# kakaobrain/rq-vae-transformer

Measured on AMD Instinct MI355X. Metric: 256x256 images/sec, AR sampling + decode (RQ-Transformer huge, 8x8x4 codes), higher is better.
Workload: dtype bf16

## Files before the change

### rq-vae-transformer_amd/csrc/conv_halo.hip

```cpp
#include <stdlib.h>
#include <type_traits>
#include "gemm.h"
#include "rq_common.h"
#include "vae_kernels.h"
#ifndef RQ_CONV_NT
#define RQ_CONV_NT 0
#endif
#ifndef RQ_CONVOUT_NT
#define RQ_CONVOUT_NT 0
#endif
static __device__ __forceinline__ rq_u128 ld128_act(const void* p) {
#if RQ_CONV_NT >= 2
    return ld128_nt(p);
#else
    return ld128(p);
#endif
}
static __device__ __forceinline__ void st128_act(void* p, rq_u128 v) {
#if RQ_CONV_NT >= 1
    st128_nt(p, v);
#else
    st128(p, v);
#endif
}
// ... 816 lines not shown
                for (int k = 0; k < PPT; ++k) {
                    const int it = (tap - FIRST) * PPT + k;
                    if (ptap && it < H_IT) rh[it] = halo_piece_value(rh, it);
                }
                compute(hbuf, wbuf, ky, kx, rh, -1);
            }
            store_w(wbuf ^ 1, rw[(tap + 1) % W_SETS]);
#pragma unroll
            for (int k = 0; k < PPT; ++k) {
                const int it = (tap - FIRST) * PPT + k;
                if (!(ptap && it < H_IT)) continue;
                if (h_in(it)) st128(sH + (hbuf ^ 1) * PK_PSTRIDE + h_loff(it), rh[it]);
            }
            RQ_CTP(2 + (c * 9 + tap) * 2);
            rq_syncthreads();
            RQ_CTP(3 + (c * 9 + tap) * 2);
            wbuf ^= 1;
        }
        hbuf ^= 1;
    };

    for (;;) {
        rq_opaque(tid_o);
        static_assert(CPR == 16 && NTH / CPR == HT_W && R_IT == TH, "piece k = tile row k");
        if (SUB)
            io_off0 = (unsigned)((((long)cur.img * p.H + 2 * cur.ty0 + (cur.cls >> 1)) * p.W + 2 * (cur.tx0 + (tid_o >> 4)) + (cur.cls & 1)) * p.Cout + cur.n0 + (tid_o & 15) * 8) * 2u;
        else
            io_off0 = (unsigned)((((long)cur.img * p.H + cur.ty0) * p.W + cur.tx0 + (tid_o >> 4)) * p.Cout + cur.n0 + (tid_o & 15) * 8) * 2u;
        RQ_CTP(1);
        for (int c = 0; c + 1 < NC; ++c) run_chunk(c, std::false_type{});
        run_chunk(NC - 1, std::true_type{});

        char* sT = (char*)smem + PK_P0 + (hbuf == 0 ? PK_PATCH : 0);
        const int lane_o = tid_o & 63, wave_o = tid_o >> 6, wm_o = wave_o >> 1, wn_o = wave_o & 1;
        float* sred = (float*)(sT + PK_TILE);
        if (RES) {
#pragma unroll
            for (int k = 0; k < R_IT; ++k) st128(sT + ((tid_o >> 4) + HT_W * k) * PK_LDR + (tid_o & 15) * 16, rr[k]);
            rq_syncthreads();
        }
#pragma unroll
        for (int i = 0; i < RPW; ++i) {
            const int ty = wm_o * RPW + i, tx = lane_o & 31;
            const int ml = ty * HT_W + tx;
#pragma unroll
            for (int j = 0; j < 2; ++j) {
#pragma unroll
                for (int q = 0; q < 4; ++q) {
                    const int nl = wn_o * 64 + j * 32 + 8 * q + 4 * (lane_o >> 5);
                    float v[4];
#pragma unroll
                    for (int e = 0; e < 4; ++e) v[e] = acc[i][j][4 * q + e];
                    if (RES) {
                        const uint32_t* rp = (const uint32_t*)(sT + ml * PK_LDR + nl * 2);
                        const uint32_t r0 = rp[0], r1 = rp[1];
                        { float lo_, hi_; rq_unpack2(r0, lo_, hi_); v[0] += lo_; v[1] += hi_; }
                        { float lo_, hi_; rq_unpack2(r1, lo_, hi_); v[2] += lo_; v[3] += hi_; }
                    }
                    struct __attribute__((aligned(8))) u64 { uint32_t a, b; } w2;
                    w2.a = pack_bf16x2(v[0], v[1]);
                    w2.b = pack_bf16x2(v[2], v[3]);
                    *(u64*)(sT + ml * PK_LDR + nl * 2) = w2;
                }
            }
        }
        if (has_next) acc_from_bias(nxt.n0);
        rq_syncthreads();
        RQ_CTP(61);
        float gs_[4], gq_[4];
#pragma unroll
        for (int e = 0; e < 4; ++e) { gs_[e] = 0.f; gq_[e] = 0.f; }
#pragma unroll
        for (int k = 0; k < R_IT; ++k) {
            const rq_u128 u = ld128(sT + ((tid_o >> 4) + HT_W * k) * PK_LDR + (tid_o & 15) * 16);
            st128_act((char*)p.out + (io_off0 + (unsigned)k * io_step), u);
            if (p.stats) rq_stats_piece(u, gs_, gq_);
        }
        if (p.stats) {
            const int gsz = p.Cout / 32;
            float a0, q0, a1, q1;
            if (gsz == 4) {
                a0 = gs_[0] + gs_[1]; q0 = gq_[0] + gq_[1];
                a1 = gs_[2] + gs_[3]; q1 = gq_[2] + gq_[3];
            } else {
                a0 = (gs_[0] + gs_[1]) + (gs_[2] + gs_[3]);
                q0 = (gq_[0] + gq_[1]) + (gq_[2] + gq_[3]);
                a1 = 0.f; q1 = 0.f;
            }
            a0 += rq_shfl_xor(a0, 16); q0 += rq_shfl_xor(q0, 16); a1 += rq_shfl_xor(a1, 16); q1 += rq_shfl_xor(q1, 16);
            a0 += rq_shfl_xor(a0, 32); q0 += rq_shfl_xor(q0, 32); a1 += rq_shfl_xor(a1, 32); q1 += rq_shfl_xor(q1, 32);
            if (lane_o < 16) {
                float* o = sred + (wave_o * 16 + lane_o) * 4;
                o[0] = a0; o[1] = q0; o[2] = a1; o[3] = q1;
            }
            rq_syncthreads();
            if (wave_o == 0) {
                const int chunk = (lane_o >> 1) & 15, pair = lane_o & 1;
                float a = 0.f, q = 0.f;
#pragma unroll
                for (int w = 0; w < NTH / 64; ++w) { a += sred[(w * 16 + chunk) * 4 + pair * 2]; q += sred[(w * 16 + chunk) * 4 + pair * 2 + 1]; }
                if (gsz == 16) {
                    a += rq_shfl_xor(a, 2);
                    q += rq_shfl_xor(q, 2);
                }
                const bool writer = gsz == 4 ? true : (gsz == 8 ? pair == 0 : (pair == 0 && (chunk & 1) == 0));
                if (writer && lane_o < 32) {
                    const int g = (cur.n0 + chunk * 8 + pair * 4) / gsz;
                    const int tiles = tiles_x * tiles_y * NCLS;
                    float* o = p.stats + (((long)cur.img * tiles + cur.trem) * 32 + g) * 2;
                    o[0] = a;
                    o[1] = q;
                }
            }
        }
        RQ_CTP(63);
#ifdef RQ_CONV_TRACE
        ++trace_tile;
#endif
        if (!has_next) break;
        rq_use(rw[1][0].x, rw[1][1].x, rw[2][0].x, rw[2][1].x);
        if (SUB) rq_use(rw[W_SETS - 1][0].x, rw[W_SETS - 1][1].x, rw[W_SETS - 1][0].y, rw[W_SETS - 1][1].y);
        rq_use(acc[0][0][0], acc[RPW - 1][1][15]);
        slot += wpx;
        cur = nxt;
        wn_cur = wn_nxt;
        if (SUB) set_class(cur.cls);
        has_next = slot_ok(slot + wpx);
        if (has_next) { nxt = decode(slot + wpx); wn_nxt = (unsigned)nxt.n0 * w_per_n + (unsigned)nxt.cls * w_per_cls; }
    }
}

struct ConvOutArgs {
    const bf16_t* x;
    const float* w;
    const float* bias;
    const float* gn;
    float* y;
    int B, H, W, Cin, Cout;
};
constexpr int OT_H = 4, OP_N = (OT_H + 2) * HP_W;
constexpr int O_NTH = 256;
constexpr int O_PLANE = OP_N * 128;

template <int FUSE_GN>
__global__ __launch_bounds__(O_NTH) void conv_out_halo_kernel(ConvOutArgs p) {
    RQ_DYN_SMEM(smem);
    const int NC = p.Cin / 64;
    char* sH = (char*)smem;
    const int wrow = 9 * p.Cin * 2 + 32;
    char* sW = sH + NC * O_PLANE;
    const int tid = threadIdx.x, lane = tid & 63, wave = rq_uniform(tid >> 6);

    const int tiles_x = p.W / HT_W, tiles_y = p.H / OT_H, tiles_img = tiles_x * tiles_y;
    const int n_mt = p.B * tiles_img;
    const int id = blockIdx.x, xcd = id & 7, slot = id >> 3, S = (int)gridDim.x >> 3;
    const int per = (n_mt + 7) >> 3;
    const int x0 = xcd * per, x1 = x0 + per < n_mt ? x0 + per : n_mt;
    const int sub = (x1 - x0 + S - 1) / (S > 0 ? S : 1);
    const int t0 = x0 + slot * sub, t1 = t0 + sub < x1 ? t0 + sub : x1;
    if (x0 >= x1 || t0 >= t1) return;

    const int cpp_sh = p.Cin == 64 ? 3 : 4;
    const int CPP = 1 << cpp_sh;
    const int cq = tid & (CPP - 1);
    const int n_piece = OP_N << cpp_sh;
    constexpr int PIT = 13;
    unsigned hyx[PIT];
#pragma unroll
    for (int k = 0; k < PIT; ++k) {
        const int q = tid + O_NTH * k;
        const int hp = q >> cpp_sh;
        const int hy = hp / HP_W, hx = hp - hy * HP_W;
        hyx[k] = q < n_piece ? (unsigned)(hy << 8 | hx) : 0xffffu;
    }
    const char* gX = (const char*)p.x;
    struct Tile { int img, ty0, tx0; };
    auto decode = [&](int t) {
        Tile d;
        d.img = t / tiles_img;
        const int trem = t - d.img * tiles_img;
        d.ty0 = (trem / tiles_x) * OT_H;
        d.tx0 = (trem - (trem / tiles_x) * tiles_x) * HT_W;
        return d;
    };
    auto request = [&](const Tile& d, rq_u128* r, f32x4* gs) {
        if (FUSE_GN) {
            const float* gn = p.gn + ((long)d.img * p.Cin + cq * 8) * 2;
#pragma unroll
            for (int e = 0; e < 4; ++e) gs[e] = *(const f32x4*)(gn + e * 4) * RQ_LOG2E;
        }
#pragma unroll
        for (int k = 0; k < PIT; ++k) {
            if (hyx[k] == 0xffffu) continue;
            const int gy = d.ty0 + (int)(hyx[k] >> 8) - 1, gx = d.tx0 + (int)(hyx[k] & 255u) - 1;
            const int cy = gy < 0 ? 0 : (gy >= p.H ? p.H - 1 : gy), cx = gx < 0 ? 0 : (gx >= p.W ? p.W - 1 : gx);
#if RQ_CONVOUT_NT
            r[k] = ld128_nt(gX + ((((long)d.img * p.H + cy) * p.W + cx) * p.Cin + cq * 8) * 2);
#else
            r[k] = ld128(gX + ((((long)d.img * p.H + cy) * p.W + cx) * p.Cin + cq * 8) * 2);
#endif
        }
    };
    auto stage = [&](const Tile& d, const rq_u128* r, const f32x4* gs) {
#pragma unroll
        for (int k = 0; k < PIT; ++k) {
            if (hyx[k] == 0xffffu) continue;
            const int hy = (int)(hyx[k] >> 8), hx = (int)(hyx[k] & 255u);
            const int gy = d.ty0 + hy - 1, gx = d.tx0 + hx - 1;
            rq_u128 v = r[k];
            if (FUSE_GN) {
                float f[8];
                rq_unpack2(v.x, f[0], f[1]);
                rq_unpack2(v.y, f[2], f[3]);
                rq_unpack2(v.z, f[4], f[5]);
                rq_unpack2(v.w, f[6], f[7]);
#pragma unroll
                for (int e = 0; e < 8; e += 2) {
                    const f32x4 ss = gs[e >> 1];
                    const float a = fmaf(f[e], ss[0], ss[1]), b = fmaf(f[e + 1], ss[2], ss[3]);
                    f[e] = rq_silu_l2(a);
                    f[e + 1] = rq_silu_l2(b);
                }
                v.x = pack_bf16x2(f[0], f[1]); v.y = pack_bf16x2(f[2], f[3]);
                v.z = pack_bf16x2(f[4], f[5]); v.w = pack_bf16x2(f[6], f[7]);
            }
            if (gy < 0 || gy >= p.H || gx < 0 || gx >= p.W) v = zero128();
            st128(sH + (unsigned)((cq >> 3) * O_PLANE) + halo_lds_off(hy, hx, cq & 7), v);
        }
    };

    rq_u128 r[PIT];
    f32x4 gs[4];
    Tile cur = decode(t0);
    request(cur, r, gs);
    const int KT = 9 * p.Cin;
    const int n_w4 = p.Cout * (KT >> 2);
    constexpr int WIT = 5;
    {
        f32x4 wr[WIT];
#pragma unroll
        for (int k = 0; k < WIT; ++k) {
            const int i = tid + O_NTH * k;
            if (i < n_w4) wr[k] = *(const f32x4*)(p.w + (long)i * 4);
        }
        stage(cur, r, gs);
#pragma unroll
        for (int k = 0; k < WIT; ++k) {
            const int i = tid + O_NTH * k;
            if (i < n_w4) {
                const int row = i / (KT >> 2), k4 = (i - row * (KT >> 2)) * 4;
                *(uint64_t*)(sW + row * wrow + k4 * 2) = (uint64_t)pack_bf16x2(wr[k][0], wr[k][1]) | ((uint64_t)pack_bf16x2(wr[k][2], wr[k][3]) << 32);
            }
        }
        for (int i = n_w4 + tid; i < 8 * (KT >> 2); i += O_NTH) {
            const int row = i / (KT >> 2), k4 = (i - row * (KT >> 2)) * 4;
            *(uint64_t*)(sW + row * wrow + k4 * 2) = 0ull;
        }
    }

    const int ftx = lane & 31, fk = lane >> 5;
    const char* wl = sW + (ftx & 7) * wrow + fk * 16;
    float bias_r[4];
#pragma unroll
    for (int co = 0; co < 4; ++co) bias_r[co] = co < p.Cout ? p.bias[co] : 0.f;
    for (int t = t0; t < t1; ++t) {
        const bool more = t + 1 < t1;
        Tile nxt = cur;
        if (more) { nxt = decode(t + 1); request(nxt, r, gs); }
        rq_syncthreads();
        f32x16 acc;
#pragma unroll
        for (int q = 0; q < 16; ++q) acc[q] = 0.f;
        constexpr int OD = 4;
        for (int c = 0; c < NC; ++c) {
            bf16x8 af[OD + 1], wf[OD + 1];
            auto frag = [&](int s, bf16x8& a, bf16x8& w) {
                const int tap = s >> 2, ks = s & 3, ky = tap / 3, kx = tap - ky * 3;
                const unsigned ha = (unsigned)(c * O_PLANE) + halo_lds_off(wave + ky, ftx + kx, fk);
                a = as_bf16x8(ld128(sH + (ha ^ (unsigned)(ks << 5))));
                w = as_bf16x8(ld128(wl + (tap * p.Cin + c * 64) * 2 + ks * 32));
            };
#pragma unroll
            for (int s = 0; s < OD; ++s) frag(s, af[s], wf[s]);
#pragma unroll
            for (int s = 0; s < 36; ++s) {
                if (s + OD < 36) frag(s + OD, af[(s + OD) % (OD + 1)], wf[(s + OD) % (OD + 1)]);
                acc = rq_mfma_32x32x16_bf16(wf[s % (OD + 1)], af[s % (OD + 1)], acc);
                rq_sched_barrier();
            }
        }
        if (lane < 32) {
            const int oy = cur.ty0 + wave, ox = cur.tx0 + lane;
#pragma unroll
            for (int co = 0; co < 4; ++co)
                if (co < p.Cout) p.y[(((long)cur.img * p.Cout + co) * p.H + oy) * p.W + ox] = acc[co] + bias_r[co];
        }
        if (!more) break;
        rq_syncthreads();
        stage(nxt, r, gs);
        cur = nxt;
    }
}

bool rq_conv_out_halo_supported(int H, int W, int Cin, int Cout) {
    return H % OT_H == 0 && W % HT_W == 0 && (Cin == 64 || Cin == 128) && Cout >= 1 && Cout <= 4;
}

int rq_launch_conv_out_halo(const bf16_t* x, const float* w, const float* bias, const float* gn, float* y, int B, int H, int W,
                            int Cin, int Cout, hipStream_t s) {
    if (!rq_conv_out_halo_supported(H, W, Cin, Cout)) return rq_fail(RQAMD_ERR_UNSUPPORTED, "conv_out_halo: shape %dx%d %d->%d", H, W, Cin, Cout);
    ConvOutArgs a{};
    a.x = x; a.w = w; a.bias = bias; a.gn = gn; a.y = y; a.B = B; a.H = H; a.W = W; a.Cin = Cin; a.Cout = Cout;
    const size_t smem = (size_t)(Cin / 64) * O_PLANE + 8 * (size_t)(9 * Cin * 2 + 32);
    static RqDeviceOnce attr_once;
    if (attr_once.first()) {
        (void)hipFuncSetAttribute((const void*)conv_out_halo_kernel<0>, hipFuncAttributeMaxDynamicSharedMemorySize, 160 * 1024);
        (void)hipFuncSetAttribute((const void*)conv_out_halo_kernel<1>, hipFuncAttributeMaxDynamicSharedMemorySize, 160 * 1024);
    }
    const int n_mt = B * (H / OT_H) * (W / HT_W);
    int nblocks = 8 * ((n_mt + 7) / 8);
    int cus = 256;
    (void)hipDeviceGetAttribute(&cus, hipDeviceAttributeMultiprocessorCount, 0);
    if (nblocks > 2 * cus) nblocks = 2 * cus / 8 * 8;
    if (const char* e = getenv("RQAMD_CONV_OUT_WGS")) {
        const int v = atoi(e) / 8 * 8;
        if (v >= 8 && v < nblocks) nblocks = v;
    }
    if (gn) RQ_LAUNCH(conv_out_halo_kernel<1>, dim3(nblocks), dim3(O_NTH), smem, s, a);
    else RQ_LAUNCH(conv_out_halo_kernel<0>, dim3(nblocks), dim3(O_NTH), smem, s, a);
    return rq_check_launch("conv_out_halo_kernel");
}

struct ConvInArgs {
    const float* x;
    const float* w;
    const float* bias;
    bf16_t* y;
    float* stats;
    int B, H, W;
};
constexpr int CI_COUT = 128, CI_PATCH = 3 * (HT_H + 2) * HP_W;
constexpr int CI_WROW = 80;
constexpr int CI_STG = 32 * (CI_COUT * 2 + 16);

__global__ __launch_bounds__(256) void conv_in_mfma_kernel(ConvInArgs p) {
    RQ_DYN_SMEM(smem);
    float* sP = (float*)smem;
    int* sK = (int*)(smem + 4096);
    char* sWt = (char*)smem + 4096 + 128;
    char* sO = sWt + CI_COUT * CI_WROW;
    const int tid = threadIdx.x, lane = tid & 63, wave = rq_uniform(tid >> 6);
    const int tiles_x = p.W / HT_W, tiles_y = p.H / HT_H;
    const int tile = blockIdx.x;
    const int img = tile / (tiles_y * tiles_x), trem = tile - img * (tiles_y * tiles_x);
    const int ty0 = (trem / tiles_x) * HT_H, tx0 = (trem - (trem / tiles_x) * tiles_x) * HT_W;

    for (int i = tid; i < CI_PATCH + 4; i += 256) {
        float v = 0.f;
        if (i < CI_PATCH) {
            const int ci = i / ((HT_H + 2) * HP_W), r = i - ci * ((HT_H + 2) * HP_W);
            const int hy = r / HP_W, hx = r - hy * HP_W;
            const int gy = ty0 + hy - 1, gx = tx0 + hx - 1;
            if (gy >= 0 && gy < p.H && gx >= 0 && gx < p.W) v = p.x[(((long)img * 3 + ci) * p.H + gy) * p.W + gx];
        }
        sP[i] = v;
    }
    if (tid < 32) {
        const int k = tid, tap = k / 3, ci = k - tap * 3, ky = tap / 3, kx = tap - ky * 3;
        sK[k] = k < 27 ? ci * ((HT_H + 2) * HP_W) + ky * HP_W + kx : -1;
    }
    for (int i = tid; i < CI_COUT * 16; i += 256) {
        const int co = i >> 4, k2 = (i & 15) * 2;
        const float a = k2 < 27 ? p.w[k2 * CI_COUT + co] : 0.f, b = k2 + 1 < 27 ? p.w[(k2 + 1) * CI_COUT + co] : 0.f;
        *(uint32_t*)(sWt + co * CI_WROW + k2 * 2) = pack_bf16x2(a, b);
    }
    rq_syncthreads();

    const int px = lane & 31, g = lane >> 5;
    int koff[2][8];
#pragma unroll
    for (int ks = 0; ks < 2; ++ks)
#pragma unroll
        for (int e = 0; e < 8; ++e) koff[ks][e] = sK[ks * 16 + g * 8 + e];
    bf16x8 bfr[2][4];
#pragma unroll
    for (int ks = 0; ks < 2; ++ks)
#pragma unroll
        for (int j = 0; j < 4; ++j) bfr[ks][j] = as_bf16x8(ld128(sWt + (j * 32 + px) * CI_WROW + (ks * 16 + g * 8) * 2));
    char* stg = sO + wave * CI_STG;
    float gs_[4] = {0.f, 0.f, 0.f, 0.f}, gq_[4] = {0.f, 0.f, 0.f, 0.f};
#pragma unroll 1
    for (int i = 0; i < 2; ++i) {
        const int row = wave * 2 + i;
        f32x16 acc[4];
#pragma unroll
        for (int j = 0; j < 4; ++j)
#pragma unroll
            for (int r = 0; r < 16; ++r) acc[j][r] = 0.f;
#pragma unroll
        for (int ks = 0; ks < 2; ++ks) {
            float f[8];
#pragma unroll
            for (int e = 0; e < 8; ++e) f[e] = koff[ks][e] >= 0 ? sP[koff[ks][e] + row * HP_W + px] : 0.f;
            rq_u128 u;
            u.x = pack_bf16x2(f[0], f[1]); u.y = pack_bf16x2(f[2], f[3]);
            u.z = pack_bf16x2(f[4], f[5]); u.w = pack_bf16x2(f[6], f[7]);
            const bf16x8 af = as_bf16x8(u);
#pragma unroll
            for (int j = 0; j < 4; ++j) acc[j] = rq_mfma_32x32x16_bf16(bfr[ks][j], af, acc[j]);
        }
#pragma unroll
        for (int j = 0; j < 4; ++j)
#pragma unroll
            for (int q = 0; q < 4; ++q) {
                const int co = j * 32 + 8 * q + 4 * g;
                const f32x4 bv = *(const f32x4*)(p.bias + co);
                struct __attribute__((aligned(8))) u64 { uint32_t a, b; } w2;
                w2.a = pack_bf16x2(acc[j][4 * q] + bv[0], acc[j][4 * q + 1] + bv[1]);
                w2.b = pack_bf16x2(acc[j][4 * q + 2] + bv[2], acc[j][4 * q + 3] + bv[3]);
                *(u64*)(stg + px * (CI_COUT * 2 + 16) + co * 2) = w2;
            }
        rq_syncthreads();
        const long pix0 = ((long)img * p.H + ty0 + row) * p.W + tx0;
#pragma unroll
        for (int k = 0; k < 8; ++k) {
            const int c = lane + 64 * k, opx = c >> 4, part = c & 15;
            const rq_u128 u = ld128(stg + opx * (CI_COUT * 2 + 16) + part * 16);
            st128(p.y + (pix0 + opx) * CI_COUT + part * 8, u);
            if (p.stats) rq_stats_piece(u, gs_, gq_);
        }
        rq_syncthreads();
    }
    if (p.stats) {
        float a0 = gs_[0] + gs_[1], q0 = gq_[0] + gq_[1], a1 = gs_[2] + gs_[3], q1 = gq_[2] + gq_[3];
        a0 += rq_shfl_xor(a0, 16); q0 += rq_shfl_xor(q0, 16); a1 += rq_shfl_xor(a1, 16); q1 += rq_shfl_xor(q1, 16);
        a0 += rq_shfl_xor(a0, 32); q0 += rq_shfl_xor(q0, 32); a1 += rq_shfl_xor(a1, 32); q1 += rq_shfl_xor(q1, 32);
        float* sred = (float*)sO;
        if (lane < 16) {
            float* o = sred + (wave * 16 + lane) * 4;
            o[0] = a0; o[1] = q0; o[2] = a1; o[3] = q1;
        }
        rq_syncthreads();
        if (tid < 32) {
            const int chunk = tid >> 1, pair = tid & 1;
            float a = 0.f, q = 0.f;
#pragma unroll
            for (int w = 0; w < 4; ++w) { a += sred[(w * 16 + chunk) * 4 + pair * 2]; q += sred[(w * 16 + chunk) * 4 + pair * 2 + 1]; }
            float* o = p.stats + (((long)img * (tiles_y * tiles_x) + trem) * 32 + tid) * 2;
            o[0] = a;
            o[1] = q;
        }
    }
}

bool rq_conv_in_mfma_supported(int H, int W, int Cin, int Cout) {
    return Cin == 3 && Cout == CI_COUT && H % HT_H == 0 && W % HT_W == 0;
}

int rq_launch_conv_in_mfma(const float* x, const float* w, const float* bias, bf16_t* y, float* stats, int B, int H, int W, hipStream_t s) {
    ConvInArgs a{};
    a.x = x; a.w = w; a.bias = bias; a.y = y; a.stats = stats; a.B = B; a.H = H; a.W = W;
    const size_t smem = 4096 + 128 + (size_t)CI_COUT * CI_WROW + 4 * (size_t)CI_STG;
    static RqDeviceOnce attr_once;
    if (attr_once.first()) {
        (void)hipFuncSetAttribute((const void*)conv_in_mfma_kernel, hipFuncAttributeMaxDynamicSharedMemorySize, (int)smem);
    }
    RQ_LAUNCH(conv_in_mfma_kernel, dim3((unsigned)(B * (H / HT_H) * (W / HT_W))), dim3(256), smem, s, a);
    return rq_check_launch("conv_in_mfma_kernel");
}

__global__ __launch_bounds__(256) void gn_params_kernel(const float* part, const float* gamma, const float* beta, float* gn, int B, int HW,
                                                        int C, int nchunk, float eps) {
    __shared__ float sa[8][32], sq[8][32], smean[32], srstd[32];
    const int b = blockIdx.x, tid = threadIdx.x, g = tid & 31, sl = tid >> 5;
    float a = 0.f, q = 0.f;
    for (int c = sl; c < nchunk; c += 8) {
        const float* o = part + (((long)b * nchunk + c) * 32 + g) * 2;
        a += o[0];
        q += o[1];
    }
    sa[sl][g] = a;
    sq[sl][g] = q;
    rq_syncthreads();
    if (tid < 32) {
        float ta = 0.f, tq = 0.f;
#pragma unroll
        for (int k = 0; k < 8; ++k) { ta += sa[k][tid]; tq += sq[k][tid]; }
        const float n = (float)HW * (float)(C / 32);
        const float mean = ta / n;
        float var = tq / n - mean * mean;
        if (var < 0.f) var = 0.f;
        smean[tid] = mean;
        srstd[tid] = 1.0f / sqrtf(var + eps);
    }
    rq_syncthreads();
    const int cpg = C / 32;
    for (int ch = tid; ch < C; ch += 256) {
        const int gg = ch / cpg;
        const float sc = srstd[gg] * gamma[ch];
        gn[((long)b * C + ch) * 2] = sc;
        gn[((long)b * C + ch) * 2 + 1] = beta[ch] - smean[gg] * sc;
    }
}

__global__ void ups_subpixel_weights_kernel(const bf16_t* w, bf16_t* wsub, int Cout, int Cin) {
    const long n = (long)4 * Cout * 4 * Cin;
    const long gid = (long)blockIdx.x * blockDim.x + threadIdx.x;
    if (gid >= n) return;
    const int ci = (int)(gid % Cin);
    long r = gid / Cin;
    const int tap = (int)(r & 3); r >>= 2;
    const int co = (int)(r % Cout);
    const int cls = (int)(r / Cout);
    const int py = cls >> 1, px = cls & 1, a = tap >> 1, b = tap & 1;
    const int ky_lo = py == 0 ? (a == 0 ? 0 : 1) : (a == 0 ? 0 : 2), ky_hi = py == 0 ? (a == 0 ? 0 : 2) : (a == 0 ? 1 : 2);
    const int kx_lo = px == 0 ? (b == 0 ? 0 : 1) : (b == 0 ? 0 : 2), kx_hi = px == 0 ? (b == 0 ? 0 : 2) : (b == 0 ? 1 : 2);
    float acc = 0.f;
    for (int ky = ky_lo; ky <= ky_hi; ++ky)
        for (int kx = kx_lo; kx <= kx_hi; ++kx) acc += bf16_to_f32(w[(((long)co * 3 + ky) * 3 + kx) * Cin + ci]);
    wsub[gid] = f32_to_bf16(acc);
}
int rq_launch_ups_subpixel_weights(const bf16_t* w, bf16_t* wsub, int Cout, int Cin, hipStream_t s) {
    const long n = (long)16 * Cout * Cin;
    RQ_LAUNCH(ups_subpixel_weights_kernel, dim3((unsigned)((n + 255) / 256)), dim3(256), 0, s, w, wsub, Cout, Cin);
    return rq_check_launch("ups_subpixel_weights_kernel");
}
bool rq_conv_halo_subpixel_supported(int H, int W, int Cin, int Cout) {
    return rq_conv_halo_supported(H, W, Cin, Cout) && (H >> 1) % HT_H == 0 && (W >> 1) % HT_W == 0;
}

bool rq_conv_halo_supported(int H, int W, int Cin, int Cout) {
    return H % HT_H == 0 && W % HT_W == 0 && Cin % 64 == 0 && Cout % H_BN == 0 && H >= 32 && H * W <= 65536;
}

int rq_conv_halo_stat_tiles(int H, int W) { return (H / HT_H) * (W / HT_W); }
static int g_conv_halo_dbg_pk = 0;
static int g_conv_halo_dbg_wpx = 0;
static bool halo_persistent(int ups) {
    static const int env = getenv("RQAMD_HALO_PERSIST") ? atoi(getenv("RQAMD_HALO_PERSIST")) : -1;
    if (g_conv_halo_dbg_pk) return g_conv_halo_dbg_pk > 0;
    return env < 0 ? ups != 0 : env != 0;
}

static int launch_conv_halo_th(const ConvHaloArgs& a, int ups, hipStream_t s) {
    constexpr int TH = HT_H, NTHR = 512;
    constexpr size_t smem = H_SMEM_BYTES;
    static_assert((size_t)TH * HT_W * (H_BN * 2 + 16) + 4096 <= H_SMEM_BYTES, "the epilogue tile overlays the operand buffers");
    static RqDeviceOnce attr_once;
    if (attr_once.first()) {
        (void)hipFuncSetAttribute((const void*)conv3x3_halo_kernel<0, 0, 0>, hipFuncAttributeMaxDynamicSharedMemorySize, (int)smem);
        (void)hipFuncSetAttribute((const void*)conv3x3_halo_kernel<0, 0, 1>, hipFuncAttributeMaxDynamicSharedMemorySize, (int)smem);
        (void)hipFuncSetAttribute((const void*)conv3x3_halo_kernel<1, 0, 0>, hipFuncAttributeMaxDynamicSharedMemorySize, (int)smem);
        (void)hipFuncSetAttribute((const void*)conv3x3_halo_kernel<1, 0, 1>, hipFuncAttributeMaxDynamicSharedMemorySize, (int)smem);
        (void)hipFuncSetAttribute((const void*)conv3x3_halo_kernel<0, 1, 0>, hipFuncAttributeMaxDynamicSharedMemorySize, (int)smem);
    }
    const int n_mt = a.B * (a.H / TH) * (a.W / HT_W), NT = a.Cout / H_BN;
    const int nblocks = 8 * ((n_mt + 7) / 8) * NT;
    if (ups == 2) {
        static RqDeviceOnce sub_once;
        static int cus_per_xcd_s[16];
        int dev = 0;
        (void)hipGetDevice(&dev);
        if (sub_once.first()) {
            (void)hipFuncSetAttribute((const void*)conv3x3_halo_pk_kernel<0, 2, 0>, hipFuncAttributeMaxDynamicSharedMemorySize, PK_SMEM);
            int cus = 0;
            if (hipDeviceGetAttribute(&cus, hipDeviceAttributeMultiprocessorCount, dev) != hipSuccess || cus < 8) cus = 256;
            cus_per_xcd_s[dev & 15] = cus / 8;
        }
        const int n_sub = a.B * ((a.H >> 1) / TH) * ((a.W >> 1) / HT_W) * 4;
        const int slots = ((n_sub + 7) / 8) * NT;
        int wpx = g_conv_halo_dbg_wpx > 0 ? g_conv_halo_dbg_wpx : cus_per_xcd_s[dev & 15];
        if (wpx > slots) wpx = slots;
        RQ_LAUNCH((conv3x3_halo_pk_kernel<0, 2, 0>), dim3(8 * wpx), dim3(512), PK_SMEM, s, a, wpx);
        return rq_check_launch("conv3x3_halo_pk_kernel<subpixel>");
    }
    if (ups && halo_persistent(ups)) {
        static RqDeviceOnce pk_once;
        static int cus_per_xcd[16];
        int dev = 0;
        (void)hipGetDevice(&dev);
        if (pk_once.first()) {
            (void)hipFuncSetAttribute((const void*)conv3x3_halo_pk_kernel<0, 1, 0>, hipFuncAttributeMaxDynamicSharedMemorySize, PK_SMEM);
            int cus = 0;
            if (hipDeviceGetAttribute(&cus, hipDeviceAttributeMultiprocessorCount, dev) != hipSuccess || cus < 8) cus = 256;
            cus_per_xcd[dev & 15] = cus / 8;
        }
        const int slots = ((n_mt + 7) / 8) * NT;
        int wpx = g_conv_halo_dbg_wpx > 0 ? g_conv_halo_dbg_wpx : cus_per_xcd[dev & 15];
        if (wpx > slots) wpx = slots;
        RQ_LAUNCH((conv3x3_halo_pk_kernel<0, 1, 0>), dim3(8 * wpx), dim3(512), PK_SMEM, s, a, wpx);
        return rq_check_launch("conv3x3_halo_pk_kernel");
    }
    if (ups) RQ_LAUNCH((conv3x3_halo_kernel<0, 1, 0>), dim3(nblocks), dim3(NTHR), smem, s, a);
    else if (a.gn && a.resid) RQ_LAUNCH((conv3x3_halo_kernel<1, 0, 1>), dim3(nblocks), dim3(NTHR), smem, s, a);
    else if (a.gn) RQ_LAUNCH((conv3x3_halo_kernel<1, 0, 0>), dim3(nblocks), dim3(NTHR), smem, s, a);
    else if (a.resid) RQ_LAUNCH((conv3x3_halo_kernel<0, 0, 1>), dim3(nblocks), dim3(NTHR), smem, s, a);
    else RQ_LAUNCH((conv3x3_halo_kernel<0, 0, 0>), dim3(nblocks), dim3(NTHR), smem, s, a);
    return rq_check_launch("conv3x3_halo_kernel");
}

int rq_launch_conv_halo(const bf16_t* x, const bf16_t* w, const float* bias, const float* gn, const bf16_t* resid, bf16_t* out,
                        float* stats, int B, int H, int W, int Cin, int Cout, int ups, hipStream_t s) {
    if (stats && Cout != 128 && Cout != 256 && Cout != 512) return rq_fail(RQAMD_ERR_UNSUPPORTED, "conv_halo: fused statistics need Cout 128/256/512");
    if (!rq_conv_halo_supported(H, W, Cin, Cout)) return rq_fail(RQAMD_ERR_UNSUPPORTED, "conv_halo: shape %dx%d %d->%d", H, W, Cin, Cout);
    if (ups && (gn || resid)) return rq_fail(RQAMD_ERR_UNSUPPORTED, "conv_halo: the upsample conv takes no GroupNorm / residual");
    if (ups == 2 && !rq_conv_halo_subpixel_supported(H, W, Cin, Cout)) return rq_fail(RQAMD_ERR_UNSUPPORTED, "conv_halo: sub-pixel form at %dx%d", H, W);
    if (2.0 * B * H * W * (Cin > Cout ? Cin : Cout) >= 4294967296.0) return rq_fail(RQAMD_ERR_UNSUPPORTED, "conv_halo: tensor larger than 4 GiB");
    ConvHaloArgs a{};
    a.x = x; a.w = w; a.bias = bias; a.gn = gn; a.resid = resid; a.out = out; a.stats = stats; a.B = B; a.H = H; a.W = W; a.Cin = Cin; a.Cout = Cout;
    return launch_conv_halo_th(a, ups, s);
}

int rq_launch_gn_params(const bf16_t* x, float* part, const float* gamma, const float* beta, float* gn, int B, int HW, int C,
                        int nchunk_have, hipStream_t s) {
    int nchunk = nchunk_have;
    if (nchunk <= 0) RQ_TRY(rq_launch_gn_stats(x, part, B, HW, C, &nchunk, s));
    RQ_LAUNCH(gn_params_kernel, dim3(B), dim3(256), 0, s, part, gamma, beta, gn, B, HW, C, nchunk, 1e-6f);
    return rq_check_launch("gn_params_kernel");
}

extern "C" int rqamd_dbg_conv_halo_bf16(const void* x, const void* w, const float* bias, const float* gn, const void* resid,
                                        int B, int H, int W, int Cin, int Cout, int ups, void* out, float* stats, void* stream) {
    if (!x || !w || !bias || !out) return rq_fail(RQAMD_ERR_INVALID, "dbg_conv_halo: null argument");
    g_conv_halo_dbg_pk = (ups & 16) ? 1 : (ups & 32) ? -1 : 0;
    g_conv_halo_dbg_wpx = (ups >> 8) & 0xff;
    const int rc = rq_launch_conv_halo((const bf16_t*)x, (const bf16_t*)w, bias, gn, (const bf16_t*)resid, (bf16_t*)out, stats, B, H, W,
                                       Cin, Cout, (ups & 64) ? 2 : (ups & 1), (hipStream_t)stream);
    g_conv_halo_dbg_pk = 0;
    g_conv_halo_dbg_wpx = 0;
// ... 27 lines not shown
```

Measured before the change: 1637.

## Add tap-batched conv_out kernel computing per-tap partials via MFMA then summing

Adds a new final-conv kernel that treats the 9 taps × Cout outputs as the MFMA M dimension. Each halo pixel is multiplied once against all tap weights, the per-tap partials go to LDS, and each output is then a sum of 9 shifted partials. This avoids the sparse MFMA use of the old kernel, which wasted most of the 32-wide output dimension when Cout ≤ 4. The new kernel also uses a rolling ring of halo rows, reloading only new rows for vertically consecutive tiles. It is on by default when 9*Cout ≤ 32, at the cost of extra LDS traffic for the partials and a serial reduction step.

```diff
diff --git a/rq-vae-transformer_amd/csrc/conv_halo.hip b/rq-vae-transformer_amd/csrc/conv_halo.hip
--- a/rq-vae-transformer_amd/csrc/conv_halo.hip
+++ b/rq-vae-transformer_amd/csrc/conv_halo.hip
@@ -1142,6 +1142,184 @@
     }
 }
 
+#ifndef RQ_CONVOUT_TAPS_TH
+#define RQ_CONVOUT_TAPS_TH 4
+#endif
+constexpr int TT_H = RQ_CONVOUT_TAPS_TH, TP_N = (TT_H + 2) * HP_W;
+constexpr int T_PLANE = TP_N * 128;
+constexpr int T_NBLK = (TP_N + 31) / 32;
+constexpr int T_PPITCH = T_NBLK * 32, T_PROWS = 28;
+static_assert(TT_H % 4 == 0, "an output row per wavefront and pass");
+
+template <int FUSE_GN, int CIN>
+__global__ __launch_bounds__(O_NTH) void conv_out_taps_kernel(ConvOutArgs p) {
+    RQ_DYN_SMEM(smem);
+    constexpr int NC = CIN / 64, NKS = CIN / 16;
+    char* sH = (char*)smem;
+    float* sP = (float*)(sH + NC * T_PLANE);
+    const int tid = threadIdx.x, lane = tid & 63, wave = rq_uniform(tid >> 6);
+
+    const int tiles_x = p.W / HT_W, tiles_y = p.H / TT_H, tiles_img = tiles_x * tiles_y;
+    const int n_mt = p.B * tiles_img;
+    const int id = blockIdx.x, xcd = id & 7, slot = id >> 3, S = (int)gridDim.x >> 3;
+    const int per = (n_mt + 7) >> 3;
+    const int x0 = xcd * per, x1 = x0 + per < n_mt ? x0 + per : n_mt;
+    const int sub = (x1 - x0 + S - 1) / (S > 0 ? S : 1);
+    const int t0 = x0 + slot * sub, t1 = t0 + sub < x1 ? t0 + sub : x1;
+    if (x0 >= x1 || t0 >= t1) return;
+
+    constexpr int cpp_sh = CIN == 64 ? 3 : 4, CPP = 1 << cpp_sh;
+    const int cq = tid & (CPP - 1);
+    constexpr int n_piece = TP_N << cpp_sh;
+    constexpr int PIT = (n_piece + O_NTH - 1) / O_NTH;
+    unsigned hyx[PIT];
+#pragma unroll
+    for (int k = 0; k < PIT; ++k) {
+        const int q = tid + O_NTH * k;
+        const int hp = q >> cpp_sh;
+        const int hy = hp / HP_W, hx = hp - hy * HP_W;
+        hyx[k] = q < n_piece ? (unsigned)(hy << 8 | hx) : 0xffffu;
+    }
+    const char* gX = (const char*)p.x;
+    constexpr int PH = TT_H + 2;
+    struct Tile { int img, ty0, tx0, rb, cont; };
+    auto decode = [&](int t, int rb_prev) {
+        Tile d;
+        d.img = t / tiles_img;
+        const int trem = t - d.img * tiles_img;
+        const int tx = trem / tiles_y, ty = trem - tx * tiles_y;
+        d.ty0 = ty * TT_H;
+        d.tx0 = tx * HT_W;
+        d.cont = t > t0 && ty > 0;
+        d.rb = d.cont ? (rb_prev + TT_H) % PH : 0;
+        return d;
+    };
+    auto request = [&](const Tile& d, rq_u128* r, f32x4* gs) {
+        if (FUSE_GN) {
+            const float* gn = p.gn + ((long)d.img * CIN + cq * 8) * 2;
+#pragma unroll
+            for (int e = 0; e < 4; ++e) gs[e] = *(const f32x4*)(gn + e * 4) * RQ_LOG2E;
+        }
+#pragma unroll
+        for (int k = 0; k < PIT; ++k) {
+            if (hyx[k] == 0xffffu || (d.cont && hyx[k] < 0x200u)) continue;
+            const int gy = d.ty0 + (int)(hyx[k] >> 8) - 1, gx = d.tx0 + (int)(hyx[k] & 255u) - 1;
+            const int cy = gy < 0 ? 0 : (gy >= p.H ? p.H - 1 : gy), cx = gx < 0 ? 0 : (gx >= p.W ? p.W - 1 : gx);
+#if RQ_CONVOUT_NT
+            r[k] = ld128_nt(gX + ((((long)d.img * p.H + cy) * p.W + cx) * CIN + cq * 8) * 2);
+#else
+            r[k] = ld128(gX + ((((long)d.img * p.H + cy) * p.W + cx) * CIN + cq * 8) * 2);
+#endif
+        }
+    };
+    auto stage = [&](const Tile& d, const rq_u128* r, const f32x4* gs) {
+#pragma unroll
+        for (int k = 0; k < PIT; ++k) {
+            if (hyx[k] == 0xffffu || (d.cont && hyx[k] < 0x200u)) continue;
+            const int hy = (int)(hyx[k] >> 8), hx = (int)(hyx[k] & 255u);
+            const int gy = d.ty0 + hy - 1, gx = d.tx0 + hx - 1;
+            const int sl = d.rb + hy < PH ? d.rb + hy : d.rb + hy - PH;
+            rq_u128 v = r[k];
+            if (FUSE_GN) {
+                float f[8];
+                rq_unpack2(v.x, f[0], f[1]);
+                rq_unpack2(v.y, f[2], f[3]);
+                rq_unpack2(v.z, f[4], f[5]);
+                rq_unpack2(v.w, f[6], f[7]);
+#pragma unroll
+                for (int e = 0; e < 8; e += 2) {
+                    const f32x4 ss = gs[e >> 1];
+                    const float a = fmaf(f[e], ss[0], ss[1]), b = fmaf(f[e + 1], ss[2], ss[3]);
+                    f[e] = rq_silu_l2(a);
+                    f[e + 1] = rq_silu_l2(b);
+                }
+                v.x = pack_bf16x2(f[0], f[1]); v.y = pack_bf16x2(f[2], f[3]);
+                v.z = pack_bf16x2(f[4], f[5]); v.w = pack_bf16x2(f[6], f[7]);
+            }
+            if (gy < 0 || gy >= p.H || gx < 0 || gx >= p.W) v = zero128();
+            st128(sH + (unsigned)((cq >> 3) * T_PLANE) + halo_lds_off(sl, hx, cq & 7), v);
+        }
+    };
+
+    rq_u128 r[PIT];
+    f32x4 gs[4];
+    Tile cur = decode(t0, 0);
+    request(cur, r, gs);
+    const int ftx = lane & 31, fk = lane >> 5;
+    bf16x8 wfrag[NKS];
+    {
+        const int wtap = ftx / p.Cout, wco = ftx - wtap * p.Cout;
+        const bool real = ftx < 9 * p.Cout;
+        const float* wl = p.w + (long)(wco * 9 + (real ? wtap : 0)) * CIN + fk * 8;
+#pragma unroll
+        for (int ks = 0; ks < NKS; ++ks) {
+            rq_u128 u = zero128();
+            if (real) {
+                const f32x4 a = *(const f32x4*)(wl + ks * 16), b = *(const f32x4*)(wl + ks * 16 + 4);
+                u.x = pack_bf16x2(a[0], a[1]); u.y = pack_bf16x2(a[2], a[3]);
+                u.z = pack_bf16x2(b[0], b[1]); u.w = pack_bf16x2(b[2], b[3]);
+            }
+            wfrag[ks] = as_bf16x8(u);
+        }
+    }
+    float bias_r[2];
+#pragma unroll
+    for (int j = 0; j < 2; ++j) bias_r[j] = fk + 2 * j < p.Cout ? p.bias[fk + 2 * j] : 0.f;
+    stage(cur, r, gs);
+
+    for (int t = t0; t < t1; ++t) {
+        const bool more = t + 1 < t1;
+        Tile nxt = cur;
+        if (more) { nxt = decode(t + 1, cur.rb); request(nxt, r, gs); }
+        rq_syncthreads();
+#pragma unroll 1
+        for (int blk = wave; blk < T_NBLK; blk += O_NTH / 64) {
+            int hp = blk * 32 + ftx;
+            hp = hp < TP_N ? hp : TP_N - 1;
+            const int hy = hp / HP_W, hx = hp - hy * HP_W;
+            const unsigned ha = halo_lds_off(cur.rb + hy < PH ? cur.rb + hy : cur.rb + hy - PH, hx, fk);
+            bf16x8 xf[NKS];
+#pragma unroll
+            for (int ks = 0; ks < NKS; ++ks) xf[ks] = as_bf16x8(ld128(sH + (unsigned)((ks >> 2) * T_PLANE) + (ha ^ (unsigned)((ks & 3) << 5))));
+            f32x16 acc;
+#pragma unroll
+            for (int q = 0; q < 16; ++q) acc[q] = 0.f;
+            rq_sched_barrier();
+#pragma unroll
+            for (int ks = 0; ks < NKS; ++ks) acc = rq_mfma_32x32x16_bf16(wfrag[ks], xf[ks], acc);
+            float* pw = sP + blk * 32 + ftx;
+#pragma unroll
+            for (int q = 0; q < 16; ++q)
+                if (q < 12 || fk == 0) pw[((q >> 2) * 8 + fk * 4 + (q & 3)) * T_PPITCH] = acc[q];
+        }
+        rq_syncthreads();
+        if (more) stage(nxt, r, gs);
+#pragma unroll
+        for (int ry = 0; ry < TT_H; ry += O_NTH / 64) {
+            const int row = ry + wave;
+            const int oy = cur.ty0 + row, ox = cur.tx0 + ftx;
+#pragma unroll
+            for (int j = 0; j < 2; ++j) {
+                const int co = fk + 2 * j;
+                if (co < p.Cout) {
+                    const float* pr = sP + co * T_PPITCH + row * HP_W + ftx;
+                    float s = pr[0];
+#pragma unroll
+                    for (int tap = 1; tap < 9; ++tap) s += pr[tap * p.Cout * T_PPITCH + (tap / 3) * HP_W + (tap % 3)];
+                    p.y[(((long)cur.img * p.Cout + co) * p.H + oy) * p.W + ox] = s + bias_r[j];
+                }
+            }
+        }
+        cur = nxt;
+    }
+}
+
+static bool conv_out_taps_selected(int Cout) {
+    if (9 * Cout > 32) return false;
+    const char* e = getenv("RQAMD_CONV_OUT_TAPS");
+    return !(e && atoi(e) == 0);
+}
+
 bool rq_conv_out_halo_supported(int H, int W, int Cin, int Cout) {
     return H % OT_H == 0 && W % HT_W == 0 && (Cin == 64 || Cin == 128) && Cout >= 1 && Cout <= 4;
 }
@@ -1151,20 +1329,37 @@
     if (!rq_conv_out_halo_supported(H, W, Cin, Cout)) return rq_fail(RQAMD_ERR_UNSUPPORTED, "conv_out_halo: shape %dx%d %d->%d", H, W, Cin, Cout);
     ConvOutArgs a{};
     a.x = x; a.w = w; a.bias = bias; a.gn = gn; a.y = y; a.B = B; a.H = H; a.W = W; a.Cin = Cin; a.Cout = Cout;
-    const size_t smem = (size_t)(Cin / 64) * O_PLANE + 8 * (size_t)(9 * Cin * 2 + 32);
+    const bool taps = conv_out_taps_selected(Cout) && H % TT_H == 0;
+    const size_t smem = taps ? (size_t)(Cin / 64) * T_PLANE + (size_t)T_PROWS * T_PPITCH * sizeof(float)
+                             : (size_t)(Cin / 64) * O_PLANE + 8 * (size_t)(9 * Cin * 2 + 32);
     static RqDeviceOnce attr_once;
     if (attr_once.first()) {
         (void)hipFuncSetAttribute((const void*)conv_out_halo_kernel<0>, hipFuncAttributeMaxDynamicSharedMemorySize, 160 * 1024);
         (void)hipFuncSetAttribute((const void*)conv_out_halo_kernel<1>, hipFuncAttributeMaxDynamicSharedMemorySize, 160 * 1024);
-    }
-    const int n_mt = B * (H / OT_H) * (W / HT_W);
+        (void)hipFuncSetAttribute((const void*)conv_out_taps_kernel<0, 64>, hipFuncAttributeMaxDynamicSharedMemorySize, 160 * 1024);
+        (void)hipFuncSetAttribute((const void*)conv_out_taps_kernel<1, 64>, hipFuncAttributeMaxDynamicSharedMemorySize, 160 * 1024);
+        (void)hipFuncSetAttribute((const void*)conv_out_taps_kernel<0, 128>, hipFuncAttributeMaxDynamicSharedMemorySize, 160 * 1024);
+        (void)hipFuncSetAttribute((const void*)conv_out_taps_kernel<1, 128>, hipFuncAttributeMaxDynamicSharedMemorySize, 160 * 1024);
+    }
+    const int n_mt = B * (H / (taps ? TT_H : OT_H)) * (W / HT_W);
     int nblocks = 8 * ((n_mt + 7) / 8);
     int cus = 256;
     (void)hipDeviceGetAttribute(&cus, hipDeviceAttributeMultiprocessorCount, 0);
-    if (nblocks > 2 * cus) nblocks = 2 * cus / 8 * 8;
+    const int per_cu = taps && TT_H > 4 ? 1 : 2;
+    if (nblocks > per_cu * cus) nblocks = per_cu * cus / 8 * 8;
     if (const char* e = getenv("RQAMD_CONV_OUT_WGS")) {
         const int v = atoi(e) / 8 * 8;
         if (v >= 8 && v < nblocks) nblocks = v;
+    }
+    if (taps) {
+        if (Cin == 64) {
+            if (gn) RQ_LAUNCH((conv_out_taps_kernel<1, 64>), dim3(nblocks), dim3(O_NTH), smem, s, a);
+            else RQ_LAUNCH((conv_out_taps_kernel<0, 64>), dim3(nblocks), dim3(O_NTH), smem, s, a);
+        } else {
+            if (gn) RQ_LAUNCH((conv_out_taps_kernel<1, 128>), dim3(nblocks), dim3(O_NTH), smem, s, a);
+            else RQ_LAUNCH((conv_out_taps_kernel<0, 128>), dim3(nblocks), dim3(O_NTH), smem, s, a);
+        }
+        return rq_check_launch("conv_out_taps_kernel");
     }
     if (gn) RQ_LAUNCH(conv_out_halo_kernel<1>, dim3(nblocks), dim3(O_NTH), smem, s, a);
     else RQ_LAUNCH(conv_out_halo_kernel<0>, dim3(nblocks), dim3(O_NTH), smem, s, a);
```

Result: no change. 1647, median of 6 (+0.6%).
